# Vandermode/TFPnP

Measured on AMD Instinct MI355X. Metric: PnP-ADMM iters/sec (and images/sec) at env_batch=48, 256x256, 30 inner iters, higher is better.
Workload: dtype f32 (v_mfma_f32_32x32x2_f32; Winograd F(2x2,3x3) on the layers with cout % 32 == 0); 1 GPU; CS-MRI ADMM 256x256 env_batch=48/GPU radial x4 sigma_n=15, 6 solver calls x 5 inner iters + PSNR reward, no early stop; global_batch=48, parallelism=single GPU

## Files before the change

### tfpnp_amd/csrc/conv3x3_wino8.hip

```cpp
#include <cmath>
#include <utility>
#include <vector>

#include "common.h"
#include "conv3x3.h"
#include "wino_common.h"

namespace pnpx {

namespace {

using namespace wino;

template <int CT_>
struct Cfg8 {
  static constexpr int CT = CT_;
  static constexpr int CK = (CT == 64) ? 16 : 8;
  static constexpr int HALVES = CK / 8;
  static constexpr int KS = CK / 2;
  static constexpr int RS = (CT == 64) ? 1 : 2;
  static constexpr int NSTG = 4 / RS;
  static constexpr int NPOS = 2 * RS;
  static constexpr int NM = NPOS * KS;
  static_assert(NM == 16, "the side-work schedule below is written for 16 MFMA slots per stage");
  static constexpr int RPXW = (CT == 64) ? 16 : 32;
  static constexpr int TX = RPXW / 2, NT = 8 * TX;
  static constexpr int RW = RPXW + 2, RPX = 18 * RW;
  static constexpr int RPXL = (CT == 64) ? 328 : RPX;
  static constexpr int RAW_ELEMS = CK * RPXL;
  static constexpr int RAW_INSTR = (RAW_ELEMS + 63) / 64;
  static constexpr int RAW_BYTES = RAW_INSTR * 256;
  static constexpr int RAW_PER_WAVE = (RAW_INSTR + 7) / 8;
  static constexpr int NRAW = RAW_INSTR / 8;
  static constexpr int UQ = 16 * CK * CT;
  static constexpr int USTG = RS * UQ;
  static constexpr int NUW = USTG / 8192;
  static constexpr int VROW = 16384;
  static constexpr int VSTG = RS * VROW;
  static constexpr int OFF_U = 0, OFF_V = 4 * USTG, OFF_RAW = OFF_V + 2 * VSTG;
  static constexpr int LDS_USED = OFF_RAW + 2 * RAW_BYTES;
  static constexpr int BAR = 12;
  static constexpr int NR = 11, NQP = (CT == 64) ? 12 : 20;
  static constexpr int QPLANE = NR * NQP * 16;
  static constexpr int ST_ELEMS = CK * NR * NQP;
  static constexpr int ST_INSTR = (ST_ELEMS + 63) / 64;
  static constexpr int ST_STRIDE = ST_INSTR * 256;
  static constexpr int ST_PER_WAVE = (ST_INSTR + 7) / 8, NSW = ST_INSTR / 8;
  static constexpr int OFF_ST = LDS_USED, OFF_TAB = OFF_ST + 2 * ST_STRIDE;
  static constexpr int LDS_USED_UPS = OFF_TAB + (18 + RW) * 16;
  static constexpr int NPOSI = 18 * RW;
};
constexpr int LDS_REQ8 = 160 * 1024;

#define WINO8_ACC \
  "a0", "a1", "a2", "a3", "a4", "a5", "a6", "a7", "a8", "a9", "a10", "a11", "a12", "a13", "a14", "a15", "a16", "a17", \
  "a18", "a19", "a20", "a21", "a22", "a23", "a24", "a25", "a26", "a27", "a28", "a29", "a30", "a31", "a32", "a33", \
  "a34", "a35", "a36", "a37", "a38", "a39", "a40", "a41", "a42", "a43", "a44", "a45", "a46", "a47", "a48", "a49", \
  "a50", "a51", "a52", "a53", "a54", "a55", "a56", "a57", "a58", "a59", "a60", "a61", "a62", "a63", "a64", "a65", \
  "a66", "a67", "a68", "a69", "a70", "a71", "a72", "a73", "a74", "a75", "a76", "a77", "a78", "a79", "a80", "a81", \
  "a82", "a83", "a84", "a85", "a86", "a87", "a88", "a89", "a90", "a91", "a92", "a93", "a94", "a95", "a96", "a97", \
  "a98", "a99", "a100", "a101", "a102", "a103", "a104", "a105", "a106", "a107", "a108", "a109", "a110", "a111", "a112", \
  "a113", "a114", "a115", "a116", "a117", "a118", "a119", "a120", "a121", "a122", "a123", "a124", "a125", "a126", "a127"
#ifdef WINO8_PRIO
#define WINO8_PRIO_UP "s_setprio 3\n\t"
#define WINO8_PRIO_DOWN "\n\ts_setprio 0"
#else
#define WINO8_PRIO_UP
#define WINO8_PRIO_DOWN
#endif
#define WINO8_MFMA(IDX, x, y) \
  asm volatile(WINO8_PRIO_UP "v_mfma_f32_32x32x2_f32 a[%2:%3], %0, %1, a[%2:%3]" WINO8_PRIO_DOWN ::"v"(x), "v"(y), "n"(16 * (IDX)), "n"(16 * (IDX) + 15) : WINO8_ACC)
#define WINO8_MFMA_FROM_ZERO(IDX, x, y) \
  asm volatile(WINO8_PRIO_UP "v_mfma_f32_32x32x2_f32 a[%2:%3], %0, %1, 0" WINO8_PRIO_DOWN ::"v"(x), "v"(y), "n"(16 * (IDX)), "n"(16 * (IDX) + 15) : WINO8_ACC)

#ifndef WINO8_ABL
#define WINO8_ABL 0
#endif
#ifdef WINO8_TRACE
__device__ unsigned long long wino8_trace_buf[2][2048];
__device__ __forceinline__ void wino8_stamp(int wave, int lane, int& n, int tag) {
  if (blockIdx.x == 0 && (wave & 3) == 0 && n < 2047) {
    const unsigned long long t = __builtin_readcyclecounter();
    if (lane == 0) wino8_trace_buf[wave >> 2][n] = (t << 8) | (unsigned)tag;
    n = __builtin_amdgcn_readfirstlane(n + 1);
    if (lane == 0) wino8_trace_buf[wave >> 2][2047] = n;
  }
}
#define WINO8_STAMP(tag) wino8_stamp(wave, lane, trace_n, tag)
#else
#define WINO8_STAMP(tag)
#endif

template <bool RAWDMA_, bool STDMA_, int IQ_>
struct StageKind {
  static constexpr bool RAWDMA = RAWDMA_, STDMA = STDMA_;
  static constexpr int IQ = IQ_;
};

using I0 = std::integral_constant<int, 0>;
using I1 = std::integral_constant<int, 1>;
using I2 = std::integral_constant<int, 2>;
using I3 = std::integral_constant<int, 3>;
using Yes = std::true_type;
using No = std::false_type;

template <int CT, bool FUSE_OUTC, bool RES, bool UPS, bool KSPLIT>
__global__ __launch_bounds__(512, 1) void conv3x3_wino8_f32_kernel(WinoArgs a) {
  static_assert(!FUSE_OUTC || CT == 32, "the fused out-conv needs all 32 couts of a pixel in one SIMD's wave pair");
  static_assert(!UPS || (!FUSE_OUTC && !RES), "the up-sampling instances are the UNet's plain decoder entries");
  static_assert(!KSPLIT || (CT == 64 && !FUSE_OUTC && !RES && !UPS), "K-split: the plain 64-cout instance (the deep levels' layers)");
  using C = Cfg8<CT>;
  constexpr int CK = C::CK, HALVES = C::HALVES, KS = C::KS, RS = C::RS, NSTG = C::NSTG, NPOS = C::NPOS;
  constexpr int TX = C::TX, NT = C::NT, RW = C::RW, RPX = C::RPX, RPXL = C::RPXL;
  constexpr int RAW_BYTES = C::RAW_BYTES, RAW_PER_WAVE = C::RAW_PER_WAVE;
  constexpr int UQ = C::UQ, USTG = C::USTG, NUW = C::NUW, VROW = C::VROW, VSTG = C::VSTG;
  constexpr int OFF_U = C::OFF_U, OFF_V = C::OFF_V, OFF_RAW = C::OFF_RAW, BAR = C::BAR;
  extern __shared__ __attribute__((aligned(16))) char lds[];
  const int tid = threadIdx.x, lane = tid & 63;
  const int wave = __builtin_amdgcn_readfirstlane(tid >> 6);
#ifdef WINO8_TRACE
  int trace_n = 0;
#endif
  const int sw = wave & 3;
  const int HpWp = a.Hp * a.Wp;
  const unsigned lds0 = (unsigned)(size_t)(lptr_t)lds;
  const int nregions = a.rx * a.ry * a.B;
  const int nx = (gridDim.x % 8 == 0 && nregions >= 32) ? 8 : 1;
  const int xcd = blockIdx.x % nx, slot = blockIdx.x / nx, nslot = gridDim.x / nx;

  struct Tile {
    int ct, b, x0, y0;
    const float* s0;
    const float* s1;
    const float* w;
    const float* s1u;
    int ok, rlo;
    int clo, c0;
    int item, g;
  };
  const int hpwp_lo = UPS ? (a.ups_h + 2) * (a.ups_w + 2 * PADL) : 0;
  auto decode = [&](int k) {
    Tile T;
    const int j = slot + nslot * k;
    const int vnct = KSPLIT ? a.nct * a.ksplit : a.nct;
    const int q = j / vnct;
    const int v = j - q * vnct;
    T.g = KSPLIT ? v / a.nct : 0;
    T.ct = KSPLIT ? v - T.g * a.nct : v;
    T.c0 = KSPLIT ? T.g * a.nch : 0;
    const int reg = nx * q + xcd;
    T.ok = reg < nregions;
    T.item = reg * a.nct + T.ct;
    T.rlo = T.clo = 0;
    T.s1u = nullptr;
    const int t1 = reg / a.rx;
    const int tx = reg - t1 * a.rx;
    const int t2 = t1 / a.ry;
    const int ty = t1 - t2 * a.ry;
    T.b = t2;
    T.x0 = tx * C::RPXW;
    T.y0 = ty * 16;
    const size_t pix = (size_t)T.y0 * a.Wp + T.x0 + (PADL - 1);
    T.s0 = a.in0 + (size_t)T.b * a.C0 * HpWp + pix;
    T.s1 = a.in1 + ((long long)T.b * a.C1 - a.C0) * (long long)HpWp + (long long)pix;
    T.w = a.u + ((size_t)T.ct * (KSPLIT ? a.nch_all : a.nch) + T.c0) * 4 * (UQ / 4);
    if (UPS) {
      const int ya = T.y0 > 0 ? T.y0 - 1 : 0, xa = T.x0 > 0 ? T.x0 - 1 : 0;
      const int rl = (int)(a.ups_sy * (float)ya), cl = (int)(a.ups_sx * (float)xa);
      const int rmax = a.ups_h + 1 - C::NR, cmax = a.ups_w + PADL - C::NQP;
      T.rlo = rl < rmax ? rl : rmax;
      T.clo = cl < cmax ? cl : cmax;
      T.s1u = a.in1 + ((long long)T.b * a.C1 - a.C0) * (long long)hpwp_lo + (long long)(T.rlo + 1) * (a.ups_w + 2 * PADL) + T.clo + PADL;
    }
    return T;
  };
  auto raw_of = [&](const Tile& X, int c) {
    const int ca = KSPLIT ? c + X.c0 : c;
    return ((CK * ca < a.C0) ? X.s0 : X.s1) + (size_t)CK * ca * HpWp;
  };

  const int wm = (CT == 64) ? (sw & 1) : 0, wn = (CT == 64) ? (sw >> 1) : sw;
  const int l31 = lane & 31, kg = lane >> 5;
  const int a_lane = ((kg * HALVES) * CT + wm * 32 + l31) * 16;
  const int b_lane = ((kg * HALVES) * NT + wn * 32 + l31) * 16;
  asm volatile("" ::: WINO8_ACC);

  auto wait_lds = [&]() { asm volatile("s_waitcnt lgkmcnt(0)" ::: "memory"); };
  auto barrier = [&]() { __builtin_amdgcn_s_barrier(); };
  auto sync_all = [&]() {
    asm volatile("s_waitcnt vmcnt(0) lgkmcnt(0)" ::: "memory");
    __builtin_amdgcn_s_barrier();
  };

  auto body = [&](auto role_tag) {
    constexpr int P = decltype(role_tag)::value;

    unsigned roff[RAW_PER_WAVE];
#pragma unroll
    for (int k = 0; k < RAW_PER_WAVE; ++k) {
      const int idx = (wave + 8 * k) * 64 + lane;
      const int c = idx / RPXL, r = idx - c * RPXL;
      const int hy = r / RW, hx = r - hy * RW;
      roff[k] = (c < CK && r < RPX) ? 4u * (unsigned)(c * HpWp + hy * a.Wp + hx) : 0u;
    }
    const unsigned uoff = lane * 16u;
    auto dma_u = [&](const float* src, int uslot) {
      if (WINO8_ABL & 4) return;
      const float* s = src + wave * 256;
#pragma unroll
      for (int k = 0; k < NUW; ++k) glds16(s + k * 2048, uoff, lds0 + OFF_U + uslot * USTG + (wave + 8 * k) * 1024);
    };
    auto dma_raw = [&](const float* src, int rbuf, int k0, int k1) {
      if (WINO8_ABL & 4) return;
      const unsigned dst = lds0 + OFF_RAW + rbuf * RAW_BYTES + wave * 256;
#pragma unroll
      for (int k = k0; k < k1; ++k)
        if (k < RAW_PER_WAVE) {
          if (k < C::NRAW || wave + 8 * k < C::RAW_INSTR) glds4(src, roff[k], dst + k * 2048);
        }
    };

    constexpr int NR = C::NR, NQP = C::NQP, QPLANE = C::QPLANE, ST_STRIDE = C::ST_STRIDE, SPW = C::ST_PER_WAVE;
    constexpr int OFF_ST = C::OFF_ST, OFF_TAB = C::OFF_TAB, NPOSI = C::NPOSI;
    unsigned soff[UPS ? SPW : 1];
    if (UPS) {
      const int wp_lo = a.ups_w + 2 * PADL;
#pragma unroll
      for (int k = 0; k < SPW; ++k) {
        const int idx = (wave + 8 * k) * 64 + lane;
        const int e = idx & 3, g = idx >> 2;
        const int q = g % NQP, g2 = g / NQP;
        const int rr = g2 % NR, Q = g2 / NR;
        soff[k] = (Q < CK / 4) ? 4u * (unsigned)((4 * Q + e) * hpwp_lo + rr * wp_lo + q) : 0u;
      }
    }
    auto dma_st = [&](const float* src, int sbuf) {
      if (!UPS || (WINO8_ABL & 4)) return;
      const unsigned dst = lds0 + OFF_ST + sbuf * ST_STRIDE + wave * 256;
#pragma unroll
      for (int k = 0; k < SPW; ++k)
        if (k < C::NSW || wave + 8 * k < C::ST_INSTR) glds4(src, soff[UPS ? k : 0], dst + k * 2048);
    };
    auto write_tables = [&](const Tile& X) {
      if (!UPS) return;
      if (tid < 18 + RW) {
        const bool row = tid < 18;
        const int i = row ? tid : tid - 18;
        const int g = (row ? X.y0 : X.x0) - 1 + i;
        const bool valid = g >= 0 && g < (row ? a.H : a.W);
        const float f = (row ? a.ups_sy : a.ups_sx) * (float)g;
        const int i0 = (int)f;
        const float l = f - (float)i0, h = 1.f - l;
        const int off = row ? (i0 - X.rlo) * NQP * 16 : (i0 - X.clo) * 16;
        f32x4 ent;
        ent[0] = __int_as_float(valid ? off : 0);
        ent[1] = valid ? h : 0.f;
        ent[2] = valid ? l : 0.f;
        ent[3] = 0.f;
        *reinterpret_cast<f32x4*>(lds + OFF_TAB + tid * 16) = ent;
      }
    };
    struct Ip {
      float hy, ly, hx, lx;
      int base;
      f32x4 v00, v01, v10, v11;
    };
    const int ipos = tid < NPOSI ? tid : NPOSI - 1;
    const int ipos_b = (512 + (tid >> 2) < NPOSI) ? 512 + (tid >> 2) : NPOSI - 1;
    auto interp_tables = [&](int pp, Ip& ip) {
      const int hyi = pp / RW, hxi = pp - hyi * RW;
      const f32x4 rt = *reinterpret_cast<const f32x4*>(lds + OFF_TAB + hyi * 16);
      const f32x4 ct = *reinterpret_cast<const f32x4*>(lds + OFF_TAB + (18 + hxi) * 16);
      ip.hy = rt[1];
      ip.ly = rt[2];
      ip.hx = ct[1];
      ip.lx = ct[2];
      ip.base = __float_as_int(rt[0]) + __float_as_int(ct[0]);
    };
    auto interp_slice = [&](auto q_tag, int sl, Ip& ip, int sbuf, int rbuf) {
      constexpr int Q = decltype(q_tag)::value;
      if (sl == 0) {
        interp_tables(ipos, ip);
      } else if (sl == 1) {
        const char* b = lds + OFF_ST + sbuf * ST_STRIDE + Q * QPLANE + ip.base;
        ip.v00 = *reinterpret_cast<const f32x4*>(b);
        ip.v01 = *reinterpret_cast<const f32x4*>(b + 16);
        ip.v10 = *reinterpret_cast<const f32x4*>(b + NQP * 16);
        ip.v11 = *reinterpret_cast<const f32x4*>(b + NQP * 16 + 16);
      } else {
        const int e = sl - 2;
        const float o = ip.hy * (ip.hx * ip.v00[e] + ip.lx * ip.v01[e]) + ip.ly * (ip.hx * ip.v10[e] + ip.lx * ip.v11[e]);
        *reinterpret_cast<float*>(lds + OFF_RAW + rbuf * RAW_BYTES + ((4 * Q + e) * RPXL + ipos) * 4) = o;
      }
    };
    auto interp_mini = [&](auto q_tag, int sl, Ip& ip, int sbuf, int rbuf) {
      constexpr int Q = decltype(q_tag)::value;
      const int e4 = (tid & 3) * 4;
      if (sl == 0) {
        interp_tables(ipos_b, ip);
      } else if (sl == 1) {
        const char* b = lds + OFF_ST + sbuf * ST_STRIDE + Q * QPLANE + ip.base + e4;
        ip.v00[0] = *reinterpret_cast<const float*>(b);
        ip.v01[0] = *reinterpret_cast<const float*>(b + 16);
        ip.v10[0] = *reinterpret_cast<const float*>(b + NQP * 16);
        ip.v11[0] = *reinterpret_cast<const float*>(b + NQP * 16 + 16);
      } else {
        const float o = ip.hy * (ip.hx * ip.v00[0] + ip.lx * ip.v01[0]) + ip.ly * (ip.hx * ip.v10[0] + ip.lx * ip.v11[0]);
        *reinterpret_cast<float*>(lds + OFF_RAW + rbuf * RAW_BYTES + (4 * Q * RPXL + ipos_b) * 4 + e4 * RPXL) = o;
      }
    };

    constexpr int TCH = (CT == 64) ? 2 : 4;
    const int cb = (CT == 64) ? (lane & 1) : 0;
    const int tt = (CT == 64) ? ((wave >> 2) * 32 + (lane >> 1)) : ((sw & 1) * 64 + lane);
    const int tkg = (CT == 64) ? (sw & 1) : (sw >> 1), thf = (CT == 64) ? (sw >> 1) : 0;
    const int tty = tt / TX, ttx = tt % TX;
    const int t_rd = (((tkg * (CK / 2) + thf * 4 + 2 * cb) * RPXL) + (2 * tty) * RW + 2 * ttx) * 4;
    const int t_wr = (((tkg * HALVES + thf) * NT) + tt) * 16 + cb * 8;
    struct Tr {
      float d[2][TCH][4];
      float r[4][TCH];
    };
    constexpr int NSL = 3 * TCH;
    auto transform_slice = [&](auto ta_tag, int sl, Tr& t, int rbuf, int vdst) {
      constexpr int A = decltype(ta_tag)::value;
      constexpr int RA = (A == 0) ? 0 : (A == 2 ? 2 : 1);
      constexpr int RB = (A == 0) ? 2 : (A == 1 ? 2 : (A == 2 ? 1 : 3));
      if (sl < TCH) {
        const int e = sl;
        const char* rb = lds + OFF_RAW + rbuf * RAW_BYTES + t_rd;
#pragma unroll
        for (int x = 0; x < 4; x += 2) {
          const f32x2 da = *reinterpret_cast<const f32x2*>(rb + (e * RPXL + RA * RW + x) * 4);
          const f32x2 db = *reinterpret_cast<const f32x2*>(rb + (e * RPXL + RB * RW + x) * 4);
          t.d[0][e][x] = da[0];
          t.d[0][e][x + 1] = da[1];
          t.d[1][e][x] = db[0];
          t.d[1][e][x + 1] = db[1];
        }
      } else if (sl < 2 * TCH) {
        const int e = sl - TCH;
#pragma unroll
        for (int x = 0; x < 4; ++x)
          t.r[x][e] = (A == 1) ? t.d[0][e][x] + t.d[1][e][x] : t.d[0][e][x] - t.d[1][e][x];
      } else if (CT == 64) {
        const int bb = (sl - 2 * TCH) >> 1, e = (sl - 2 * TCH) & 1;
        (void)e;
        if (((sl - 2 * TCH) & 1) == 0) return;
        f32x2 v;
#pragma unroll
        for (int q = 0; q < 2; ++q)
          v[q] = (bb == 0) ? t.r[0][q] - t.r[2][q] : (bb == 1) ? t.r[1][q] + t.r[2][q] : (bb == 2) ? t.r[2][q] - t.r[1][q] : t.r[1][q] - t.r[3][q];
        *reinterpret_cast<f32x2*>(lds + vdst + t_wr + bb * 4096) = v;
      } else {
        const int bb = sl - 2 * TCH;
        f32x4 v;
#pragma unroll
        for (int e = 0; e < 4; ++e)
          v[e] = (bb == 0) ? t.r[0][e] - t.r[2][e] : (bb == 1) ? t.r[1][e] + t.r[2][e] : (bb == 2) ? t.r[2][e] - t.r[1][e] : t.r[1][e] - t.r[3][e];
        *reinterpret_cast<f32x4*>(lds + vdst + t_wr + bb * 4096) = v;
      }
    };
    constexpr int NSLT = (CT == 64) ? 2 * TCH + 8 : NSL;
    auto vdst_of = [&](auto sn_tag) {
      constexpr int SN = decltype(sn_tag)::value;
      return OFF_V + ((CT == 64) ? (SN & 1) * VSTG : SN * VSTG + P * VROW);
    };

    f32x4 af[NPOS][HALVES], bf[NPOS][HALVES];
    auto read_operand = [&](auto s_tag, int uslot, int pos, int h) {
      constexpr int S = decltype(s_tag)::value;
      constexpr int VB = (CT == 64) ? (S & 1) : S;
      const int r = pos >> 1, b = 2 * P + (pos & 1);
      if (WINO8_ABL & 2) {
        af[pos][h] = bf[pos][h] = (f32x4){1.f, 1.f, 1.f, 1.f};
        return;
      }
      af[pos][h] = *reinterpret_cast<const f32x4*>(lds + OFF_U + uslot * USTG + r * UQ + b * (UQ / 4) + a_lane + h * (CT * 16));
      bf[pos][h] = *reinterpret_cast<const f32x4*>(lds + OFF_V + VB * VSTG + r * VROW + b * 4096 + b_lane + h * (NT * 16));
    };

    struct Side {
      int t_rbuf;
      int u_cur, u_next;
      const float* u_src;
      int u_dst;
      const float* raw_src;
      int raw_buf;
      const float* st_src;
      int st_buf;
      int i_sbuf, i_rbuf;
    };
    auto stage = [&](auto s_tag, auto zero_tag, auto wait_tag, auto prefetch_tag, auto kind_tag, const Side& sd) {
      using K = decltype(kind_tag);
      constexpr int S = decltype(s_tag)::value;
      constexpr bool PREFETCH = decltype(prefetch_tag)::value;
      constexpr int SN = (S + 1) % NSTG;
      constexpr bool ZERO = decltype(zero_tag)::value;
      constexpr int WAITN = decltype(wait_tag)::value;
      constexpr bool HALOST = (CT == 64) ? (S == 0) : (S == 1);
      constexpr bool RAWST = HALOST && K::RAWDMA;
      constexpr bool STST = UPS && HALOST && K::STDMA;
      constexpr int IQ = UPS ? K::IQ : -1;
      using IQt = std::integral_constant<int, IQ < 0 ? 0 : IQ>;
      Ip ipa, ipb;
      auto islice = [&](int q) {
        if (IQ >= 0) interp_slice(IQt{}, q, ipa, sd.i_sbuf, sd.i_rbuf);
      };
      auto imini = [&](int q) {
        if (IQ >= 0 && CT == 32) interp_mini(IQt{}, q, ipb, sd.i_sbuf, sd.i_rbuf);
      };
      using TA = std::integral_constant<int, (CT == 64) ? SN : 2 * SN + P>;
      using SNt = std::integral_constant<int, SN>;
      Tr t;
      auto operand = [&](int pos, int h) { read_operand(s_tag, sd.u_cur, pos, h); };
      auto tslice = [&](int q) {
        if (!(WINO8_ABL & 1)) transform_slice(TA{}, q, t, sd.t_rbuf, vdst_of(SNt{}));
      };
      auto side = [&](int sl) {
        if (CT == 64) {
          if (sl == 0) operand(0, 1);
          else if (sl == 1) operand(1, 1);
          if (sl < 2) tslice(sl);
          if (sl == 2) dma_u(sd.u_src, sd.u_dst);
          if (RAWST && sl >= 3 && sl < 9) dma_raw(sd.raw_src, sd.raw_buf, 2 * (sl - 3), 2 * (sl - 3) + 2);
          if (STST && sl == 9) dma_st(sd.st_src, sd.st_buf);
          if (IQ < 0) {
            if (sl == 4) tslice(2);
            if (sl == 5) tslice(3);
            if (sl >= 6 && sl < 10) tslice(5 + 2 * (sl - 6));
          } else {
            if (sl == 3) tslice(2), tslice(3);
            if (sl == 4) tslice(5), tslice(7);
            if (sl == 5) tslice(9), tslice(11), islice(0);
            if (sl == 6) islice(1);
            if (sl >= 8 && sl < 12) islice(2 + (sl - 8));
          }
        } else {
          if (sl == 0) tslice(0);
          else if (sl == 1) operand(2, 0);
          else if (sl == 2) tslice(1);
          else if (sl == 3) operand(3, 0);
          else if (sl == 4) tslice(4), tslice(2);
          else if (sl == 5) tslice(5), tslice(3);
          else if (sl == 6) tslice(6), tslice(7);
          else if (sl == 7) tslice(8), tslice(9), islice(0);
          else if (sl == 8) tslice(10), tslice(11), islice(1);
          else if (sl == 9) islice(2), islice(3), imini(0);
          else if (sl == 10) islice(4), islice(5), imini(1), dma_u(sd.u_src, sd.u_dst);
          else if (sl == 11) imini(2);
          if (RAWST && sl >= 6 && sl < 11) dma_raw(sd.raw_src, sd.raw_buf, 2 * (sl - 6), 2 * (sl - 6) + 2);
          if (STST && sl == 9) dma_st(sd.st_src, sd.st_buf);
        }
        if (sl == BAR) {
          if (!(WINO8_ABL & 8)) {
            WINO8_STAMP(32 + S);
            asm volatile("s_waitcnt vmcnt(%0) lgkmcnt(0)" ::"n"(WAITN) : "memory");
            WINO8_STAMP(48 + S);
            barrier();
          }
          WINO8_STAMP(S);
          if (PREFETCH) {
            read_operand(SNt{}, sd.u_next, 0, 0);
            read_operand(SNt{}, sd.u_next, 1, 0);
          }
        }
      };
#pragma unroll
      for (int pair = 0; pair < NPOS / 2; ++pair)
#pragma unroll
        for (int m = 0; m < KS; ++m)
#pragma unroll
          for (int bl = 0; bl < 2; ++bl) {
            const int pos = 2 * pair + bl;
            const int sl = pair * (2 * KS) + m * 2 + bl;
            const float x = af[pos][m >> 2][m & 3], y = bf[pos][m >> 2][m & 3];
            const bool from_zero = ZERO && m == 0;
            if (!(WINO8_ABL & 16)) switch (pos) {
              case 0: if (from_zero) WINO8_MFMA_FROM_ZERO(2 * (RS * S) + 0, x, y); else WINO8_MFMA(2 * (RS * S) + 0, x, y); break;
              case 1: if (from_zero) WINO8_MFMA_FROM_ZERO(2 * (RS * S) + 1, x, y); else WINO8_MFMA(2 * (RS * S) + 1, x, y); break;
              case 2: if (from_zero) WINO8_MFMA_FROM_ZERO((2 * (RS * S) + 2) & 7, x, y); else WINO8_MFMA((2 * (RS * S) + 2) & 7, x, y); break;
              default: if (from_zero) WINO8_MFMA_FROM_ZERO((2 * (RS * S) + 3) & 7, x, y); else WINO8_MFMA((2 * (RS * S) + 3) & 7, x, y); break;
            }
            side(sl);
            __builtin_amdgcn_sched_barrier(0);
          }
    };

    auto epilogue = [&](const Tile& T, int xsend, int xrecv, int zoff) {
      const int tile = wn * 32 + l31, ty = tile / TX, tx = tile % TX;
      const int cbase = T.ct * CT + wm * 32 + 4 * kg;
      float* ob = a.out + ((size_t)T.b * a.Cout) * HpWp + (size_t)(T.y0 + 2 * ty + 1) * a.Wp + T.x0 + 2 * tx + PADL;
      const int Hp_pool = padded_h(a.H / 2), Wp_pool = padded_w(a.W / 2);
      const size_t HpWp_pool = (size_t)Hp_pool * Wp_pool;
      float* pb = a.pool ? a.pool + (size_t)T.b * a.Cout * HpWp_pool + (size_t)(T.y0 / 2 + ty + 1) * Wp_pool + T.x0 / 2 + tx + PADL : nullptr;
      constexpr int R0 = 8 * P;
      constexpr int RX = 8 - R0;
      WINO8_STAMP(16);
      asm volatile("s_nop 15\n\ts_nop 15" ::: "memory", WINO8_ACC);
      float bias_r[8];
#pragma unroll
      for (int j = 0; j < 8; ++j) bias_r[j] = a.bias[cbase + ((R0 + j) & 3) + 8 * ((R0 + j) >> 2)];
      auto column_sums = [&](auto r_tag) {
        constexpr int R = decltype(r_tag)::value;
        f32x4 sv;
        static_for<2>([&](auto bl_tag) {
          constexpr int BL = decltype(bl_tag)::value;
          float m0, m1, m2, m3;
          asm volatile("v_accvgpr_read_b32 %0, a[%1]" : "=v"(m0) : "n"(16 * (0 + BL) + R) : WINO8_ACC);
          asm volatile("v_accvgpr_read_b32 %0, a[%1]" : "=v"(m1) : "n"(16 * (2 + BL) + R) : WINO8_ACC);
          asm volatile("v_accvgpr_read_b32 %0, a[%1]" : "=v"(m2) : "n"(16 * (4 + BL) + R) : WINO8_ACC);
          asm volatile("v_accvgpr_read_b32 %0, a[%1]" : "=v"(m3) : "n"(16 * (6 + BL) + R) : WINO8_ACC);
          sv[BL] = (m0 + m1) + m2;
          sv[2 + BL] = (m1 - m2) - m3;
        });
        return sv;
      };
      f32x4 theirs[8];
      {
        char* xs = lds + xsend + lane * 16;
        static_for<8>([&](auto j_tag) {
          *reinterpret_cast<f32x4*>(xs + decltype(j_tag)::value * 1024) = column_sums(std::integral_constant<int, RX + decltype(j_tag)::value>{});
        });
        wait_lds();
        barrier();
        WINO8_STAMP(17);
        const char* xr = lds + xrecv + lane * 16;
#pragma unroll
        for (int j = 0; j < 8; ++j) theirs[j] = *reinterpret_cast<const f32x4*>(xr + j * 1024);
      }
      f32x2 rs0[RES ? 4 : 1], rs1[RES ? 4 : 1];
      auto load_res = [&](int j0) {
        const float* rb = a.res + (ob - a.out);
#pragma unroll
        for (int q = 0; q < 4; ++q) {
          const float* rp = rb + (size_t)(cbase + ((R0 + j0 + q) & 3) + 8 * ((R0 + j0 + q) >> 2)) * HpWp;
          rs0[RES ? q : 0] = *reinterpret_cast<const f32x2*>(rp);
          rs1[RES ? q : 0] = *reinterpret_cast<const f32x2*>(rp + a.Wp);
        }
      };
      float ow[8];
      float s00 = 0.f, s01 = 0.f, s10 = 0.f, s11 = 0.f;
      if (FUSE_OUTC) {
#pragma unroll
        for (int j = 0; j < 8; ++j) ow[j] = a.outc_w[cbase + ((R0 + j) & 3) + 8 * ((R0 + j) >> 2)];
      }
      wait_lds();
      float* const part_tile = KSPLIT ? a.part + ((size_t)T.item * a.ksplit * 8 + wave) * 2048 + lane * 4 : nullptr;
      float* const part_mine = KSPLIT ? part_tile + (size_t)T.g * (8 * 2048) : nullptr;
      static_for<8>([&](auto j_tag) {
        constexpr int j = decltype(j_tag)::value;
        constexpr int R = R0 + j;
        if (RES && (j & 3) == 0) load_res(j);
        const int co = cbase + (R & 3) + 8 * (R >> 2);
        const f32x4 mine = column_sums(std::integral_constant<int, R>{});
        const f32x4 lo = (P == 0) ? mine : theirs[j], hi = (P == 0) ? theirs[j] : mine;
        const float bias = bias_r[j];
        float y00 = (lo[0] + lo[1]) + hi[0], y01 = (lo[1] - hi[0]) - hi[1];
        float y10 = (lo[2] + lo[3]) + hi[2], y11 = (lo[3] - hi[2]) - hi[3];
        if (KSPLIT) {
          *reinterpret_cast<f32x4*>(part_mine + j * 256) = (f32x4){y00, y01, y10, y11};
          return;
        }
        y00 += bias;
        y01 += bias;
        y10 += bias;
        y11 += bias;
        y00 = fmaxf(y00, y00 * a.slope);
        y01 = fmaxf(y01, y01 * a.slope);
        y10 = fmaxf(y10, y10 * a.slope);
        y11 = fmaxf(y11, y11 * a.slope);
        if (RES) {
          const f32x2 r0 = rs0[RES ? (j & 3) : 0], r1 = rs1[RES ? (j & 3) : 0];
          if (a.res_mask) {
            y00 *= r0[0] > 0.f ? 1.f : a.mask_slope;
            y01 *= r0[1] > 0.f ? 1.f : a.mask_slope;
            y10 *= r1[0] > 0.f ? 1.f : a.mask_slope;
            y11 *= r1[1] > 0.f ? 1.f : a.mask_slope;
          } else {
            y00 += r0[0];
            y01 += r0[1];
            y10 += r1[0];
            y11 += r1[1];
          }
        }
        if (FUSE_OUTC) {
          s00 = fmaf(ow[j], y00, s00);
          s01 = fmaf(ow[j], y01, s01);
          s10 = fmaf(ow[j], y10, s10);
          s11 = fmaf(ow[j], y11, s11);
        } else {
          float* o = ob + (size_t)co * HpWp;
          *reinterpret_cast<f32x2*>(o) = (f32x2){y00, y01};
          *reinterpret_cast<f32x2*>(o + a.Wp) = (f32x2){y10, y11};
          if (a.pool) pb[(size_t)co * HpWp_pool] = fmaxf(fmaxf(y00, y01), fmaxf(y10, y11));
        }
      });
      WINO8_STAMP(19);
      if (FUSE_OUTC) {
        s00 += __shfl_xor(s00, 32);
        s01 += __shfl_xor(s01, 32);
        s10 += __shfl_xor(s10, 32);
        s11 += __shfl_xor(s11, 32);
        char* zb = lds + zoff + lane * 16;
        if (P == 1) {
          *reinterpret_cast<f32x4*>(zb) = (f32x4){s00, s01, s10, s11};
          wait_lds();
        }
        barrier();
        f32x4 o = {0.f, 0.f, 0.f, 0.f};
        if (P == 0) {
          o = *reinterpret_cast<const f32x4*>(zb);
          wait_lds();
        }
        barrier();
        if (P == 0) {
          s00 += o[0];
          s01 += o[1];
          s10 += o[2];
          s11 += o[3];
          const size_t px0 = ((size_t)T.b * a.H + T.y0 + 2 * ty) * a.W + T.x0 + 2 * tx;
          const float ob0 = a.outc_b[0];
          const f32x2 xi0 = *reinterpret_cast<const f32x2*>(a.x_img + px0), xi1 = *reinterpret_cast<const f32x2*>(a.x_img + px0 + a.W);
          const float v00 = xi0[0] + (s00 + ob0), v01 = xi0[1] + (s01 + ob0), v10 = xi1[0] + (s10 + ob0), v11 = xi1[1] + (s11 + ob0);
          *reinterpret_cast<f32x2*>(a.img_pre + px0) = (f32x2){v00, v01};
          *reinterpret_cast<f32x2*>(a.img_pre + px0 + a.W) = (f32x2){v10, v11};
          *reinterpret_cast<f32x2*>(a.img + px0) = (f32x2){fminf(fmaxf(v00, 0.f), 1.f), fminf(fmaxf(v01, 0.f), 1.f)};
          *reinterpret_cast<f32x2*>(a.img + px0 + a.W) = (f32x2){fminf(fmaxf(v10, 0.f), 1.f), fminf(fmaxf(v11, 0.f), 1.f)};
        }
      } else {
        barrier();
      }
      WINO8_STAMP(20);
    };

    constexpr int NST = KSPLIT ? 8 : (FUSE_OUTC ? (P == 0 ? 4 : 0) : 16);
    constexpr int NRAW = C::NRAW;

    int k = 0;
    Tile T = decode(0);
    if (!T.ok) return;
    WINO8_STAMP(14);
    if (CT == 64) {
      dma_raw(raw_of(T, 0), 0, 0, RAW_PER_WAVE);
      dma_u(T.w, 0);
      dma_u(T.w + (UQ / 4), 1);
      dma_u(T.w + 2 * (UQ / 4), 2);
    } else {
      dma_raw(T.s0, 0, 0, RAW_PER_WAVE);
      dma_raw(raw_of(T, 1), 1, 0, RAW_PER_WAVE);
      dma_u(T.w, 0);
      dma_u(T.w + (USTG / 4), 1);
      dma_u(T.w + 2 * (USTG / 4), 2);
    }
    sync_all();
    {
      Tr t;
#pragma unroll
      for (int sl = 0; sl < NSLT; ++sl) transform_slice(std::integral_constant<int, (CT == 64) ? 0 : P>{}, sl, t, 0, vdst_of(I0{}));
    }
    sync_all();
    WINO8_STAMP(15);
    read_operand(I0{}, 0, 0, 0);
    read_operand(I0{}, 0, 1, 0);

    auto chunk = [&](auto first_tag, auto k1_tag, auto k2_tag, auto k3_tag, const float* w_c, const float* nu, const float* nu2,
                     const float* nraw, const float* nst, int cc) {
      constexpr int EPI = decltype(first_tag)::value ? NST : 0;
      constexpr bool K1 = UPS && decltype(k1_tag)::value, K2 = UPS && decltype(k2_tag)::value, K3 = UPS && decltype(k3_tag)::value;
      constexpr int NSW = C::NSW;
      using Pre = Yes;
      const int rcur = cc & 1, rnext = rcur ^ 1;
      if constexpr (CT == 64) {
        using S0k = StageKind<!K1, K2, K1 ? 1 : -1>;
        using S1k = StageKind<false, false, K1 ? 2 : -1>;
        using S2k = StageKind<false, false, K1 ? 3 : -1>;
        using S3k = StageKind<false, false, K2 ? 0 : -1>;
        constexpr int HALO = (K1 ? 0 : NRAW) + (K2 ? NSW : 0);
        stage(I0{}, first_tag, std::integral_constant<int, NUW + EPI + NUW + HALO>{}, Yes{}, S0k{},
              Side{rcur, 0, 1, w_c + 3 * (UQ / 4), 3, nraw, rnext, nst, rcur, rnext, rnext});
        stage(I1{}, first_tag, std::integral_constant<int, EPI + NUW + HALO + NUW>{}, Yes{}, S1k{},
              Side{rcur, 1, 2, nu, 0, nullptr, 0, nullptr, 0, rnext, rnext});
        stage(I2{}, first_tag, std::integral_constant<int, 2 * NUW>{}, Yes{}, S2k{}, Side{rcur, 2, 3, nu + (UQ / 4), 1, nullptr, 0, nullptr, 0, rnext, rnext});
        stage(I3{}, first_tag, std::integral_constant<int, 2 * NUW>{}, Pre{}, S3k{}, Side{rnext, 3, 0, nu + 2 * (UQ / 4), 2, nullptr, 0, nullptr, 0, rcur, rcur});
      } else {
        using S0k = StageKind<false, false, K1 ? 1 : -1>;
        using S1k = StageKind<!K2, K3, K2 ? 0 : -1>;
        const int u0 = 2 * rcur, n0 = 2 * rnext;
        stage(I0{}, first_tag, std::integral_constant<int, NUW + EPI>{}, Yes{}, S0k{},
              Side{rcur, u0, u0 + 1, nu + (USTG / 4), n0 + 1, nullptr, 0, nullptr, 0, rnext, rnext});
        stage(I1{}, first_tag, std::integral_constant<int, 2 * NUW + EPI + (K2 ? 0 : NRAW) + (K3 ? NSW : 0)>{}, Pre{}, S1k{},
              Side{rnext, u0 + 1, n0, nu2, u0, nraw, rcur, nst, rnext, rcur, rcur});
      }
    };

    int cc = 0;
    for (;;) {
      Tile Tn = decode(k + 1);
      const bool more = Tn.ok;
      if (!more) Tn = T;
      for (int c = 0; c < a.nch; ++c, ++cc) {
        const float* w_c = T.w + (size_t)c * 4 * (UQ / 4);
        const float* nu = (c + 1 < a.nch) ? w_c + 4 * (UQ / 4) : Tn.w;
        const float* nu2 = (c + 2 < a.nch) ? w_c + 8 * (UQ / 4) : Tn.w + (size_t)(c + 2 - a.nch) * 4 * (UQ / 4);
        constexpr int AH = (CT == 64) ? 1 : 2;
        const float* nraw = (c + AH < a.nch) ? raw_of(T, c + AH) : raw_of(Tn, c + AH - a.nch);
        if constexpr (!UPS) {
          if (c == 0) chunk(Yes{}, No{}, No{}, No{}, w_c, nu, nu2, nraw, nullptr, cc);
          else chunk(No{}, No{}, No{}, No{}, w_c, nu, nu2, nraw, nullptr, cc);
        } else {
          const int cu = a.C0 / CK;
          auto ups = [&](int j) { return c + j < a.nch && c + j >= cu; };
          const bool k1 = ups(1), k2 = ups(2), k3 = (CT == 32) && ups(3);
          const float* nst = T.s1u + (size_t)CK * (c + AH + 1) * hpwp_lo;
          if (c == 0) {
            write_tables(T);
            chunk(Yes{}, No{}, No{}, No{}, w_c, nu, nu2, nraw, nst, cc);
          } else if constexpr (CT == 64) {
            if (!k1 && !k2) chunk(No{}, No{}, No{}, No{}, w_c, nu, nu2, nraw, nst, cc);
            else if (!k1 && k2) chunk(No{}, No{}, Yes{}, No{}, w_c, nu, nu2, nraw, nst, cc);
            else if (k1 && k2) chunk(No{}, Yes{}, Yes{}, No{}, w_c, nu, nu2, nraw, nst, cc);
            else chunk(No{}, Yes{}, No{}, No{}, w_c, nu, nu2, nraw, nst, cc);
          } else {
            if (!k1 && !k2 && !k3) chunk(No{}, No{}, No{}, No{}, w_c, nu, nu2, nraw, nst, cc);
            else if (!k1 && !k2) chunk(No{}, No{}, No{}, Yes{}, w_c, nu, nu2, nraw, nst, cc);
            else if (!k1 && k3) chunk(No{}, No{}, Yes{}, Yes{}, w_c, nu, nu2, nraw, nst, cc);
            else if (k1 && k2 && k3) chunk(No{}, Yes{}, Yes{}, Yes{}, w_c, nu, nu2, nraw, nst, cc);
            else if (k1 && k2) chunk(No{}, Yes{}, Yes{}, No{}, w_c, nu, nu2, nraw, nst, cc);
            else if (k1) chunk(No{}, Yes{}, No{}, No{}, w_c, nu, nu2, nraw, nst, cc);
            else chunk(No{}, No{}, Yes{}, No{}, w_c, nu, nu2, nraw, nst, cc);
          }
        }
      }
      const int rl = (cc - 1) & 1;
      const int bufA = (CT == 64) ? ((sw < 2) ? OFF_U + 3 * USTG + sw * 8192 : OFF_V + VSTG + (sw - 2) * 8192) : OFF_V + VSTG + sw * 8192;
      const int bufB = (CT == 64) ? ((sw < 2) ? OFF_RAW + rl * RAW_BYTES + sw * 8192 : C::LDS_USED + (sw - 2) * 8192)
                                  : ((sw < 1) ? OFF_U + (2 * rl + 1) * USTG : C::LDS_USED + (sw - 1) * 8192);
      static_assert(C::LDS_USED + (CT == 64 ? 2 : 3) * 8192 <= LDS_REQ8 && 2 * 8192 <= RAW_BYTES && USTG >= 8192, "exchange buffers");
      epilogue(T, P == 1 ? bufA : bufB, P == 1 ? bufB : bufA, bufB);
      if (!more) break;
      T = Tn;
      ++k;
    }
    sync_all();
  };

  if (wave < 4) body(I0{});
  else body(I1{});
}

__global__ __launch_bounds__(512) void wino8_ksplit_finish_kernel(WinoArgs a) {
  using C = Cfg8<64>;
  const int item = blockIdx.x, tid = threadIdx.x, lane = tid & 63, wave = tid >> 6;
  const int reg = item / a.nct, ct = item - reg * a.nct;
  const int t1 = reg / a.rx, txr = reg - t1 * a.rx, b = t1 / a.ry, tyr = t1 - b * a.ry;
  const int x0 = txr * C::RPXW, y0 = tyr * 16;
  const int P = wave >> 2, sw = wave & 3, wm = sw & 1, wn = sw >> 1, l31 = lane & 31, kg = lane >> 5;
  const int tile = wn * 32 + l31, ty = tile / C::TX, tx = tile % C::TX;
  const int cbase = ct * 64 + wm * 32 + 4 * kg;
  const size_t HpWp = (size_t)a.Hp * a.Wp;
  float* ob = a.out + ((size_t)b * a.Cout) * HpWp + (size_t)(y0 + 2 * ty + 1) * a.Wp + x0 + 2 * tx + PADL;
  const int Hp_pool = padded_h(a.H / 2), Wp_pool = padded_w(a.W / 2);
  const size_t HpWp_pool = (size_t)Hp_pool * Wp_pool;
  float* pb = a.pool ? a.pool + (size_t)b * a.Cout * HpWp_pool + (size_t)(y0 / 2 + ty + 1) * Wp_pool + x0 / 2 + tx + PADL : nullptr;
  const float* part = a.part + ((size_t)item * a.ksplit * 8 + wave) * 2048 + lane * 4;
#pragma unroll
  for (int j = 0; j < 8; ++j) {
    const int R = 8 * P + j;
    const int co = cbase + (R & 3) + 8 * (R >> 2);
    f32x4 y = *reinterpret_cast<const f32x4*>(part + j * 256);
    for (int g = 1; g < a.ksplit; ++g) {
      const f32x4 pg = *reinterpret_cast<const f32x4*>(part + (size_t)g * (8 * 2048) + j * 256);
      y[0] += pg[0];
      y[1] += pg[1];
      y[2] += pg[2];
      y[3] += pg[3];
    }
    const float bias = a.bias[co];
    float y00 = y[0] + bias, y01 = y[1] + bias, y10 = y[2] + bias, y11 = y[3] + bias;
    y00 = fmaxf(y00, y00 * a.slope);
    y01 = fmaxf(y01, y01 * a.slope);
    y10 = fmaxf(y10, y10 * a.slope);
    y11 = fmaxf(y11, y11 * a.slope);
    float* o = ob + (size_t)co * HpWp;
    *reinterpret_cast<f32x2*>(o) = (f32x2){y00, y01};
    *reinterpret_cast<f32x2*>(o + a.Wp) = (f32x2){y10, y11};
    if (a.pool) pb[(size_t)co * HpWp_pool] = fmaxf(fmaxf(y00, y01), fmaxf(y10, y11));
  }
}

}

static int wino8_ct(int C0, int C1, int cout, int H, int W) {
  if (C0 <= 0 || H < 16 || H % 16 != 0) return 0;
  if (cout % 64 == 0) return (C0 % 16 == 0 && C1 % 16 == 0 && W % 16 == 0) ? 64 : 0;
  if (cout % 32 == 0) return (C0 % 8 == 0 && C1 % 8 == 0 && W % 32 == 0 && C0 + C1 >= 16) ? 32 : 0;
  return 0;
}
bool conv3x3_wino8_ok(int C0, int C1, int cout, int H, int W) { return wino8_ct(C0, C1, cout, H, W) != 0; }

int conv3x3_wino8_ksplit(int C0, int C1, int cout, int H, int W, int rule) {
  if (wino8_ct(C0, C1, cout, H, W) != 64 || rule <= 0) return 1;
  const int t = (H / 16) * (W / 16) * (cout / 64), nch = (C0 + C1) / 16;
  const int g8 = rule == 1 ? 4 : (rule & 15), g16 = rule == 1 ? 2 : ((rule >> 4) & 15);
  int g = t <= 8 ? g8 : (t <= 16 ? g16 : 1);
  if (g != 1 && g != 2 && g != 4) g = 1;
  while (g > 1 && g * t > 32) g /= 2;
  while (g > 1 && (nch % g != 0 || nch / g < 4)) g /= 2;
  return g;
}
size_t conv3x3_wino8_ksplit_bytes_per_image() { return (size_t)32 * 8 * 2048 * sizeof(float); }

template <int CT, bool FUSE_OUTC, bool RES, bool UPS = false, bool KSPLIT = false>
static int launch_wino8(WinoArgs a, hipStream_t s) {
  using C = Cfg8<CT>;
  static_assert(C::LDS_USED <= LDS_REQ8 && C::LDS_USED_UPS <= LDS_REQ8, "LDS budget");
  a.nct = a.Cout / CT;
  a.nch = (a.C0 + a.C1) / C::CK;
  a.nch_all = a.nch;
  if (KSPLIT) a.nch /= a.ksplit;
  else a.ksplit = 1;
  a.rx = a.W / C::RPXW;
  a.ry = a.H / 16;
  static std::once_flag attr_once[64];
  int dev = 0;
  PNPX_HIP(hipGetDevice(&dev));
  if (dev >= 0 && dev < 64) {
    hipError_t e = hipSuccess;
    std::call_once(attr_once[dev], [&] {
      e = hipFuncSetAttribute(reinterpret_cast<const void*>(&conv3x3_wino8_f32_kernel<CT, FUSE_OUTC, RES, UPS, KSPLIT>), hipFuncAttributeMaxDynamicSharedMemorySize, LDS_REQ8);
    });
    PNPX_HIP(e);
  }
  const int vnct = a.nct * a.ksplit;
  const long long nreg = (long long)a.rx * a.ry * a.B, ntiles = nreg * vnct;
  long long grid = 256;
  if (grid >= ntiles) grid = ntiles;
  else if ((grid / 8) % vnct != 0 && grid >= 8LL * vnct) grid -= grid % (8 * vnct);
  hipLaunchKernelGGL((conv3x3_wino8_f32_kernel<CT, FUSE_OUTC, RES, UPS, KSPLIT>), dim3((unsigned)grid), dim3(512), LDS_REQ8, s, a);
  PNPX_LAUNCH_CHECK();
  if (KSPLIT) {
    hipLaunchKernelGGL(wino8_ksplit_finish_kernel, dim3((unsigned)(nreg * a.nct)), dim3(512), 0, s, a);
    PNPX_LAUNCH_CHECK();
  }
  return PNPX_OK;
}

int launch_conv3x3_wino8_outc(const float* u, const float* bias, const float* in0, int cin, const float* outc_w, const float* outc_b,
                              const float* x_img, float* img, float* img_pre, int B, int H, int W, hipStream_t s) {
  if (wino8_ct(cin, 0, 32, H, W) != 32) {
    set_error("conv3x3_wino8_outc: unsupported geometry (%d -> 32 channels, %d x %d)", cin, H, W);
    return PNPX_ERR_SHAPE;
  }
  WinoArgs a{};
  a.in0 = in0;
  a.in1 = in0;
  a.u = u;
  a.bias = bias;
  a.out = nullptr;
  a.outc_w = outc_w;
  a.outc_b = outc_b;
  a.x_img = x_img;
  a.img = img;
  a.img_pre = img_pre ? img_pre : img;
  a.B = B;
  a.H = H;
  a.W = W;
  a.Hp = padded_h(H);
  a.Wp = padded_w(W);
  a.C0 = cin;
  a.C1 = 0;
  a.Cout = 32;
  a.slope = 0.2f;
  return launch_wino8<32, true, false>(a, s);
}

bool conv3x3_wino8_ups_ok(int C0, int C1, int cout, int H, int W) {
  const int ct = wino8_ct(C0, C1, cout, H, W);
  if (!ct || C1 <= 0 || H % 2 || W % 2) return false;
  const int h = H / 2, w = W / 2;
  if (ct == 64) return C0 / 16 >= 3 && h + 1 >= Cfg8<64>::NR && w + PADL >= Cfg8<64>::NQP;
  return C0 / 8 >= 4 && h + 1 >= Cfg8<32>::NR && w + PADL >= Cfg8<32>::NQP;
}

int launch_conv3x3_wino8_ups(const float* u, const float* bias, int cout, const float* in0, int C0, const float* in1_lowres, int C1,
                             float* out, int B, int H, int W, hipStream_t s, float slope) {
  if (!conv3x3_wino8_ups_ok(C0, C1, cout, H, W)) {
    set_error("conv3x3_wino8_ups: unsupported geometry (%d + up(%d) -> %d channels, %d x %d)", C0, C1, cout, H, W);
    return PNPX_ERR_SHAPE;
  }
  WinoArgs a{};
  a.in0 = in0;
// ... 92 lines not shown
```

Measured before the change: 115.9 iters/s.

## Use 16-byte raw-tile DMA for CT=32 Winograd and move last-chunk halo load into epilogue

Result: no change. 114.7 iters/s (median of 2 runs) (-1.0%).

```diff
diff --git a/tfpnp_amd/csrc/conv3x3_wino8.hip b/tfpnp_amd/csrc/conv3x3_wino8.hip
--- a/tfpnp_amd/csrc/conv3x3_wino8.hip
+++ b/tfpnp_amd/csrc/conv3x3_wino8.hip
@@ -25,11 +25,19 @@
   static_assert(NM == 16, "the side-work schedule below is written for 16 MFMA slots per stage");
   static constexpr int RPXW = (CT == 64) ? 16 : 32;
   static constexpr int TX = RPXW / 2, NT = 8 * TX;
-  static constexpr int RW = RPXW + 2, RPX = 18 * RW;
+  static constexpr int WW = RPXW + 2;
+  static constexpr int RW = (CT == 64) ? WW : 40, RPX = 18 * RW;
+  static constexpr int WX = (CT == 64) ? 0 : PADL - 1;
+  static_assert(CT == 64 || ((PADL - 1 - WX) % 4 == 0 && RW % 4 == 0 && RW >= WX + WW), "the cover starts on a granule of the activation row");
   static constexpr int RPXL = (CT == 64) ? 328 : RPX;
   static constexpr int RAW_ELEMS = CK * RPXL;
-  static constexpr int RAW_INSTR = (RAW_ELEMS + 63) / 64;
-  static constexpr int RAW_BYTES = RAW_INSTR * 256;
+  static constexpr int RAW_GRAN = (CT == 64) ? 4 : 16;
+  static constexpr int RAW_INSTR = (RAW_ELEMS * 4 / RAW_GRAN + 63) / 64;
+  static constexpr int RAW_IBYTES = 64 * RAW_GRAN;
+  static constexpr int RAW_BYTES = RAW_INSTR * RAW_IBYTES;
+  static constexpr int RAW_SHIFT = (CT == 64) ? 0 : 4, RAW_TAIL = (CT == 64) ? 0 : 16;
+  static constexpr int RAW_ORG = RAW_SHIFT + 4 * WX;
+  static_assert(RAW_ORG % 16 == 0 && RAW_SHIFT <= RAW_TAIL && RPXL % 2 == 0 && RW % 2 == 0, "8-byte aligned halo reads");
   static constexpr int RAW_PER_WAVE = (RAW_INSTR + 7) / 8;
   static constexpr int NRAW = RAW_INSTR / 8;
   static constexpr int UQ = 16 * CK * CT;
@@ -38,7 +46,7 @@
   static constexpr int VROW = 16384;
   static constexpr int VSTG = RS * VROW;
   static constexpr int OFF_U = 0, OFF_V = 4 * USTG, OFF_RAW = OFF_V + 2 * VSTG;
-  static constexpr int LDS_USED = OFF_RAW + 2 * RAW_BYTES;
+  static constexpr int LDS_USED = OFF_RAW + 2 * RAW_BYTES + RAW_TAIL;
   static constexpr int BAR = 12;
   static constexpr int NR = 11, NQP = (CT == 64) ? 12 : 20;
   static constexpr int QPLANE = NR * NQP * 16;
@@ -47,8 +55,8 @@
   static constexpr int ST_STRIDE = ST_INSTR * 256;
   static constexpr int ST_PER_WAVE = (ST_INSTR + 7) / 8, NSW = ST_INSTR / 8;
   static constexpr int OFF_ST = LDS_USED, OFF_TAB = OFF_ST + 2 * ST_STRIDE;
-  static constexpr int LDS_USED_UPS = OFF_TAB + (18 + RW) * 16;
-  static constexpr int NPOSI = 18 * RW;
+  static constexpr int LDS_USED_UPS = OFF_TAB + (18 + WW) * 16;
+  static constexpr int NPOSI = 18 * WW;
 };
 constexpr int LDS_REQ8 = 160 * 1024;
 
@@ -111,7 +119,7 @@
   static_assert(!KSPLIT || (CT == 64 && !FUSE_OUTC && !RES && !UPS), "K-split: the plain 64-cout instance (the deep levels' layers)");
   using C = Cfg8<CT>;
   constexpr int CK = C::CK, HALVES = C::HALVES, KS = C::KS, RS = C::RS, NSTG = C::NSTG, NPOS = C::NPOS;
-  constexpr int TX = C::TX, NT = C::NT, RW = C::RW, RPX = C::RPX, RPXL = C::RPXL;
+  constexpr int TX = C::TX, NT = C::NT, WW = C::WW, RW = C::RW, RPX = C::RPX, RPXL = C::RPXL, RAW_ORG = C::RAW_ORG;
   constexpr int RAW_BYTES = C::RAW_BYTES, RAW_PER_WAVE = C::RAW_PER_WAVE;
   constexpr int UQ = C::UQ, USTG = C::USTG, NUW = C::NUW, VROW = C::VROW, VSTG = C::VSTG;
   constexpr int OFF_U = C::OFF_U, OFF_V = C::OFF_V, OFF_RAW = C::OFF_RAW, BAR = C::BAR;
@@ -160,7 +168,7 @@
     T.b = t2;
     T.x0 = tx * C::RPXW;
     T.y0 = ty * 16;
-    const size_t pix = (size_t)T.y0 * a.Wp + T.x0 + (PADL - 1);
+    const size_t pix = (size_t)T.y0 * a.Wp + T.x0 + (PADL - 1 - C::WX);
     T.s0 = a.in0 + (size_t)T.b * a.C0 * HpWp + pix;
     T.s1 = a.in1 + ((long long)T.b * a.C1 - a.C0) * (long long)HpWp + (long long)pix;
     T.w = a.u + ((size_t)T.ct * (KSPLIT ? a.nch_all : a.nch) + T.c0) * 4 * (UQ / 4);
@@ -198,7 +206,8 @@
     unsigned roff[RAW_PER_WAVE];
 #pragma unroll
     for (int k = 0; k < RAW_PER_WAVE; ++k) {
-      const int idx = (wave + 8 * k) * 64 + lane;
+      constexpr int EPL = C::RAW_GRAN / 4;
+      const int idx = ((wave + 8 * k) * 64 + lane) * EPL;
       const int c = idx / RPXL, r = idx - c * RPXL;
       const int hy = r / RW, hx = r - hy * RW;
       roff[k] = (c < CK && r < RPX) ? 4u * (unsigned)(c * HpWp + hy * a.Wp + hx) : 0u;
@@ -212,11 +221,14 @@
     };
     auto dma_raw = [&](const float* src, int rbuf, int k0, int k1) {
       if (WINO8_ABL & 4) return;
-      const unsigned dst = lds0 + OFF_RAW + rbuf * RAW_BYTES + wave * 256;
+      const unsigned dst = lds0 + OFF_RAW + rbuf * RAW_BYTES + C::RAW_SHIFT + wave * C::RAW_IBYTES;
 #pragma unroll
       for (int k = k0; k < k1; ++k)
         if (k < RAW_PER_WAVE) {
-          if (k < C::NRAW || wave + 8 * k < C::RAW_INSTR) glds4(src, roff[k], dst + k * 2048);
+          if (k < C::NRAW || wave + 8 * k < C::RAW_INSTR) {
+            if constexpr (CT == 64) glds4(src, roff[k], dst + k * 8 * C::RAW_IBYTES);
+            else glds16(src, roff[k], dst + k * 8 * C::RAW_IBYTES);
+          }
         }
     };
 
@@ -243,7 +255,7 @@
     };
     auto write_tables = [&](const Tile& X) {
       if (!UPS) return;
-      if (tid < 18 + RW) {
+      if (tid < 18 + WW) {
         const bool row = tid < 18;
         const int i = row ? tid : tid - 18;
         const int g = (row ? X.y0 : X.x0) - 1 + i;
@@ -265,8 +277,9 @@
       int base;
       f32x4 v00, v01, v10, v11;
     };
-    const int ipos = tid < NPOSI ? tid : NPOSI - 1;
-    const int ipos_b = (512 + (tid >> 2) < NPOSI) ? 512 + (tid >> 2) : NPOSI - 1;
+    auto ioff_of = [&](int pp) { return pp + (pp / WW) * (RW - WW); };
+    const int ipos = ioff_of(tid < NPOSI ? tid : NPOSI - 1);
+    const int ipos_b = ioff_of((512 + (tid >> 2) < NPOSI) ? 512 + (tid >> 2) : NPOSI - 1);
     auto interp_tables = [&](int pp, Ip& ip) {
       const int hyi = pp / RW, hxi = pp - hyi * RW;
       const f32x4 rt = *reinterpret_cast<const f32x4*>(lds + OFF_TAB + hyi * 16);
@@ -290,7 +303,7 @@
       } else {
         const int e = sl - 2;
         const float o = ip.hy * (ip.hx * ip.v00[e] + ip.lx * ip.v01[e]) + ip.ly * (ip.hx * ip.v10[e] + ip.lx * ip.v11[e]);
-        *reinterpret_cast<float*>(lds + OFF_RAW + rbuf * RAW_BYTES + ((4 * Q + e) * RPXL + ipos) * 4) = o;
+        *reinterpret_cast<float*>(lds + OFF_RAW + rbuf * RAW_BYTES + RAW_ORG + ((4 * Q + e) * RPXL + ipos) * 4) = o;
       }
     };
     auto interp_mini = [&](auto q_tag, int sl, Ip& ip, int sbuf, int rbuf) {
@@ -306,16 +319,16 @@
         ip.v11[0] = *reinterpret_cast<const float*>(b + NQP * 16 + 16);
       } else {
         const float o = ip.hy * (ip.hx * ip.v00[0] + ip.lx * ip.v01[0]) + ip.ly * (ip.hx * ip.v10[0] + ip.lx * ip.v11[0]);
-        *reinterpret_cast<float*>(lds + OFF_RAW + rbuf * RAW_BYTES + (4 * Q * RPXL + ipos_b) * 4 + e4 * RPXL) = o;
+        *reinterpret_cast<float*>(lds + OFF_RAW + rbuf * RAW_BYTES + RAW_ORG + (4 * Q * RPXL + ipos_b) * 4 + e4 * RPXL) = o;
       }
     };
 
     constexpr int TCH = (CT == 64) ? 2 : 4;
     const int cb = (CT == 64) ? (lane & 1) : 0;
-    const int tt = (CT == 64) ? ((wave >> 2) * 32 + (lane >> 1)) : ((sw & 1) * 64 + lane);
+    const int tt = (CT == 64) ? ((wave >> 2) * 32 + (lane >> 1)) : ((sw & 1) * 64 + (lane & 15) + 16 * (((lane >> 4) & 1) * 2 + (lane >> 5)));
     const int tkg = (CT == 64) ? (sw & 1) : (sw >> 1), thf = (CT == 64) ? (sw >> 1) : 0;
     const int tty = tt / TX, ttx = tt % TX;
-    const int t_rd = (((tkg * (CK / 2) + thf * 4 + 2 * cb) * RPXL) + (2 * tty) * RW + 2 * ttx) * 4;
+    const int t_rd = RAW_ORG + (((tkg * (CK / 2) + thf * 4 + 2 * cb) * RPXL) + (2 * tty) * RW + 2 * ttx) * 4;
     const int t_wr = (((tkg * HALVES + thf) * NT) + tt) * 16 + cb * 8;
     struct Tr {
       float d[2][TCH][4];
@@ -449,7 +462,7 @@
           else if (sl == 9) islice(2), islice(3), imini(0);
           else if (sl == 10) islice(4), islice(5), imini(1), dma_u(sd.u_src, sd.u_dst);
           else if (sl == 11) imini(2);
-          if (RAWST && sl >= 6 && sl < 11) dma_raw(sd.raw_src, sd.raw_buf, 2 * (sl - 6), 2 * (sl - 6) + 2);
+          if (RAWST && sl >= 6 && sl < 6 + RAW_PER_WAVE) dma_raw(sd.raw_src, sd.raw_buf, sl - 6, sl - 5);
           if (STST && sl == 9) dma_st(sd.st_src, sd.st_buf);
         }
         if (sl == BAR) {
@@ -487,7 +500,7 @@
           }
     };
 
-    auto epilogue = [&](const Tile& T, int xsend, int xrecv, int zoff) {
+    auto epilogue = [&](const Tile& T, int xsend, int xrecv, int zoff, const float* hsrc, int hbuf) {
       const int tile = wn * 32 + l31, ty = tile / TX, tx = tile % TX;
       const int cbase = T.ct * CT + wm * 32 + 4 * kg;
       float* ob = a.out + ((size_t)T.b * a.Cout) * HpWp + (size_t)(T.y0 + 2 * ty + 1) * a.Wp + T.x0 + 2 * tx + PADL;
@@ -631,6 +644,7 @@
       } else {
         barrier();
       }
+      if constexpr (CT == 32) dma_raw(hsrc, hbuf, 0, RAW_PER_WAVE);
       WINO8_STAMP(20);
     };
 
@@ -664,9 +678,11 @@
     read_operand(I0{}, 0, 0, 0);
     read_operand(I0{}, 0, 1, 0);
 
-    auto chunk = [&](auto first_tag, auto k1_tag, auto k2_tag, auto k3_tag, const float* w_c, const float* nu, const float* nu2,
+    auto chunk = [&](auto first_tag, auto k1_tag, auto k2_tag, auto k3_tag, auto last_tag, const float* w_c, const float* nu, const float* nu2,
                      const float* nraw, const float* nst, int cc) {
       constexpr int EPI = decltype(first_tag)::value ? NST : 0;
+      constexpr int EPI0 = (CT == 32) ? 0 : EPI;
+      constexpr bool LAST = CT == 32 && decltype(last_tag)::value;
       constexpr bool K1 = UPS && decltype(k1_tag)::value, K2 = UPS && decltype(k2_tag)::value, K3 = UPS && decltype(k3_tag)::value;
       constexpr int NSW = C::NSW;
       using Pre = Yes;
@@ -685,11 +701,11 @@
         stage(I3{}, first_tag, std::integral_constant<int, 2 * NUW>{}, Pre{}, S3k{}, Side{rnext, 3, 0, nu + 2 * (UQ / 4), 2, nullptr, 0, nullptr, 0, rcur, rcur});
       } else {
         using S0k = StageKind<false, false, K1 ? 1 : -1>;
-        using S1k = StageKind<!K2, K3, K2 ? 0 : -1>;
+        using S1k = StageKind<!K2 && !LAST, K3, K2 ? 0 : -1>;
         const int u0 = 2 * rcur, n0 = 2 * rnext;
-        stage(I0{}, first_tag, std::integral_constant<int, NUW + EPI>{}, Yes{}, S0k{},
+        stage(I0{}, first_tag, std::integral_constant<int, NUW + EPI0>{}, Yes{}, S0k{},
               Side{rcur, u0, u0 + 1, nu + (USTG / 4), n0 + 1, nullptr, 0, nullptr, 0, rnext, rnext});
-        stage(I1{}, first_tag, std::integral_constant<int, 2 * NUW + EPI + (K2 ? 0 : NRAW) + (K3 ? NSW : 0)>{}, Pre{}, S1k{},
+        stage(I1{}, first_tag, std::integral_constant<int, 2 * NUW + EPI + (K2 || LAST ? 0 : NRAW) + (K3 ? NSW : 0)>{}, Pre{}, S1k{},
               Side{rnext, u0 + 1, n0, nu2, u0, nraw, rcur, nst, rnext, rcur, rcur});
       }
     };
@@ -706,8 +722,9 @@
         constexpr int AH = (CT == 64) ? 1 : 2;
         const float* nraw = (c + AH < a.nch) ? raw_of(T, c + AH) : raw_of(Tn, c + AH - a.nch);
         if constexpr (!UPS) {
-          if (c == 0) chunk(Yes{}, No{}, No{}, No{}, w_c, nu, nu2, nraw, nullptr, cc);
-          else chunk(No{}, No{}, No{}, No{}, w_c, nu, nu2, nraw, nullptr, cc);
+          if (c == 0) chunk(Yes{}, No{}, No{}, No{}, No{}, w_c, nu, nu2, nraw, nullptr, cc);
+          else if (CT == 32 && c == a.nch - 1) chunk(No{}, No{}, No{}, No{}, std::integral_constant<bool, CT == 32>{}, w_c, nu, nu2, nraw, nullptr, cc);
+          else chunk(No{}, No{}, No{}, No{}, No{}, w_c, nu, nu2, nraw, nullptr, cc);
         } else {
           const int cu = a.C0 / CK;
           auto ups = [&](int j) { return c + j < a.nch && c + j >= cu; };
@@ -715,29 +732,31 @@
           const float* nst = T.s1u + (size_t)CK * (c + AH + 1) * hpwp_lo;
           if (c == 0) {
             write_tables(T);
-            chunk(Yes{}, No{}, No{}, No{}, w_c, nu, nu2, nraw, nst, cc);
+            chunk(Yes{}, No{}, No{}, No{}, No{}, w_c, nu, nu2, nraw, nst, cc);
           } else if constexpr (CT == 64) {
-            if (!k1 && !k2) chunk(No{}, No{}, No{}, No{}, w_c, nu, nu2, nraw, nst, cc);
-            else if (!k1 && k2) chunk(No{}, No{}, Yes{}, No{}, w_c, nu, nu2, nraw, nst, cc);
-            else if (k1 && k2) chunk(No{}, Yes{}, Yes{}, No{}, w_c, nu, nu2, nraw, nst, cc);
-            else chunk(No{}, Yes{}, No{}, No{}, w_c, nu, nu2, nraw, nst, cc);
+            if (!k1 && !k2) chunk(No{}, No{}, No{}, No{}, No{}, w_c, nu, nu2, nraw, nst, cc);
+            else if (!k1 && k2) chunk(No{}, No{}, Yes{}, No{}, No{}, w_c, nu, nu2, nraw, nst, cc);
+            else if (k1 && k2) chunk(No{}, Yes{}, Yes{}, No{}, No{}, w_c, nu, nu2, nraw, nst, cc);
+            else chunk(No{}, Yes{}, No{}, No{}, No{}, w_c, nu, nu2, nraw, nst, cc);
           } else {
-            if (!k1 && !k2 && !k3) chunk(No{}, No{}, No{}, No{}, w_c, nu, nu2, nraw, nst, cc);
-            else if (!k1 && !k2) chunk(No{}, No{}, No{}, Yes{}, w_c, nu, nu2, nraw, nst, cc);
-            else if (!k1 && k3) chunk(No{}, No{}, Yes{}, Yes{}, w_c, nu, nu2, nraw, nst, cc);
-            else if (k1 && k2 && k3) chunk(No{}, Yes{}, Yes{}, Yes{}, w_c, nu, nu2, nraw, nst, cc);
-            else if (k1 && k2) chunk(No{}, Yes{}, Yes{}, No{}, w_c, nu, nu2, nraw, nst, cc);
-            else if (k1) chunk(No{}, Yes{}, No{}, No{}, w_c, nu, nu2, nraw, nst, cc);
-            else chunk(No{}, No{}, Yes{}, No{}, w_c, nu, nu2, nraw, nst, cc);
+            if (!k1 && !k2 && !k3 && c == a.nch - 1) chunk(No{}, No{}, No{}, No{}, Yes{}, w_c, nu, nu2, nraw, nst, cc);
+            else if (!k1 && !k2 && !k3) chunk(No{}, No{}, No{}, No{}, No{}, w_c, nu, nu2, nraw, nst, cc);
+            else if (!k1 && !k2) chunk(No{}, No{}, No{}, Yes{}, No{}, w_c, nu, nu2, nraw, nst, cc);
+            else if (!k1 && k3) chunk(No{}, No{}, Yes{}, Yes{}, No{}, w_c, nu, nu2, nraw, nst, cc);
+            else if (k1 && k2 && k3) chunk(No{}, Yes{}, Yes{}, Yes{}, No{}, w_c, nu, nu2, nraw, nst, cc);
+            else if (k1 && k2) chunk(No{}, Yes{}, Yes{}, No{}, No{}, w_c, nu, nu2, nraw, nst, cc);
+            else if (k1) chunk(No{}, Yes{}, No{}, No{}, No{}, w_c, nu, nu2, nraw, nst, cc);
+            else chunk(No{}, No{}, Yes{}, No{}, No{}, w_c, nu, nu2, nraw, nst, cc);
           }
         }
       }
       const int rl = (cc - 1) & 1;
       const int bufA = (CT == 64) ? ((sw < 2) ? OFF_U + 3 * USTG + sw * 8192 : OFF_V + VSTG + (sw - 2) * 8192) : OFF_V + VSTG + sw * 8192;
       const int bufB = (CT == 64) ? ((sw < 2) ? OFF_RAW + rl * RAW_BYTES + sw * 8192 : C::LDS_USED + (sw - 2) * 8192)
-                                  : ((sw < 1) ? OFF_U + (2 * rl + 1) * USTG : C::LDS_USED + (sw - 1) * 8192);
-      static_assert(C::LDS_USED + (CT == 64 ? 2 : 3) * 8192 <= LDS_REQ8 && 2 * 8192 <= RAW_BYTES && USTG >= 8192, "exchange buffers");
-      epilogue(T, P == 1 ? bufA : bufB, P == 1 ? bufB : bufA, bufB);
+                                  : ((sw < 1) ? OFF_U + (2 * rl + 1) * USTG : (sw < 3) ? C::LDS_USED + (sw - 1) * 8192 : OFF_RAW + rl * RAW_BYTES);
+      static_assert(C::LDS_USED + 2 * 8192 <= LDS_REQ8 && (CT == 64 ? 2 : 1) * 8192 <= RAW_BYTES && USTG >= 8192, "exchange buffers");
+      static_assert(CT == 64 || (C::LDS_USED == 145424 && C::LDS_USED_UPS == 160592 && C::LDS_USED_UPS <= LDS_REQ8), "CT 32 LDS budget");
+      epilogue(T, P == 1 ? bufA : bufB, P == 1 ? bufB : bufA, bufB, CT == 64 ? nullptr : raw_of(Tn, 1), rl);
       if (!more) break;
       T = Tn;
       ++k;
```
